# ProgramerSalar/stable-diffusion-from-scratch

Measured on NVIDIA B200. Metric: 512px DDIM-50 images/sec, higher is better.
Workload: dtype bf16

## Files before the change

include/sdb200.h:

```cpp
#ifndef SDB200_H
#define SDB200_H

#include <stdint.h>

#ifdef __cplusplus
extern "C" {
#endif

#define SDB_OK            0
#define SDB_ERR_INVALID  -1
#define SDB_ERR_CUDA     -2
#define SDB_ERR_NOTMA    -3

#define SDB_F32   0
#define SDB_BF16  1

int         sdb_version(void);
const char* sdb_last_error_string(void);
int         sdb_device_sm_count(void);
unsigned long long sdb_launch_count(void);
int sdb_pdl_skip_next(int n);

int sdb_nchw_to_nhwc(const float* src, void* dst, int dst_dtype, int N, int C, int dst_C, int HW, void* stream);
int sdb_nchw_to_nhwc_split(const float* src, void* dst , int N, int C, int dst_C, int HW, void* stream);
// ... 65 lines not shown
    long long lda, ldb, ldc, ldr, ldv;
    int M, N, K;
    float alpha;
    int b_kn;
    int nb1, nb2;
    long long sa1, sa2, sb1, sb2, sc1, sc2;
    int kh, kw, stride, pad, up;
    int NB, IH, IW, Cin, OH, OW;
    int out_dtype;
} sdb_simt_args;
int sdb_simt_contract(const sdb_simt_args* args , void* stream);

typedef struct sdb_tc_args {
    const void* A; const void* B; void* out;
    const float* bias; const float* rowvec; const float* residual;
    long long lda, ldb, ldc, ldr, ldv;
    int M, N, K;
    int out_dtype;
    int geglu;
    int col_group, col_group_stride;
    int split_k;
    int block_n;
    int taps;
    int kw;
    int stride, pad_h, pad_w;
    int NB, IH, IW, Cin, OH, OW;
    int cout_pad;
    int out_sh, out_sw, out_oh, out_ow, OHF, OWF;
    void* ws; long long ws_bytes;
    int rows_per_item;
    int variant;
    float* colstats; long long colstats_slots;
    int b_const;
} sdb_tc_args;
int sdb_tc_colstats_layout(const sdb_tc_args* args , long long* slots, long long* slots_per_item);
long long sdb_tc_workspace_bytes(const sdb_tc_args* args );
int sdb_tc_contract(const sdb_tc_args* args , void* stream);
int sdb_tc_set_pair_kernel(int enable);
int sdb_tc_set_tma_epilogue(int enable);
int sdb_tc_set_tail_split(int enable);

typedef struct sdb_attn_args {
    const void* q; const void* k; const void* v; void* out;
    long long q_bs, q_ss, q_hs;
    long long k_bs, k_ss, k_hs;
    long long v_bs, v_ss, v_hs;
    long long o_bs, o_ss, o_hs;
    int B, H, Sq, Sk, d, dpad;
    float scale;
    int dense;
    int causal;
} sdb_attn_args;
int sdb_attention_fwd(const sdb_attn_args* args , void* stream);
int sdb_attention_set_short_key_kernel(int enable);

int sdb_attention_wide_fwd(const void* q, const void* k, const void* v, void* out, long long q_bs, long long q_ss,
                           long long k_bs, long long k_ss, long long v_bs, long long v_ss, long long o_bs, long long o_ss,
                           int B, int Sq, int Sk, int d, float scale, void* stream);

#define SDB_NCHW  0
#define SDB_NHWC  1
long long sdb_vq_ws_bytes(long long M, int n_e);
int sdb_vq_quantize(const float* z, int z_layout, int N, int HW, int D, const float* codebook, int n_e, float beta,
                    float* z_q, int zq_layout, long long* idx, float* loss, void* ws, int* counters, void* stream);
int sdb_vq_codebook_gather(const long long* idx, long long M, const float* codebook, int n_e, int D, float* out, int out_layout,
                           int HW, void* stream);

int sdb_patch_unfold(const float* x, int B, int C, int H, int W, int kh, int kw, int sh, int sw, float* out, void* stream);
int sdb_patch_fold(const float* o, int B, int C, int KH, int KW, int Ly, int Lx, int SH, int SW, int OH, int OW,
                   const float* wpix, const float* wcrop, int L, float* out, void* stream);

#ifdef __cplusplus
}
// ... 3 lines not shown
```

stable-diffusion-from-scratch_b200/_lib.py:

```python
import ctypes as C
import os

import torch

HERE = os.path.dirname(os.path.abspath(__file__))
LIB_PATH = os.path.join(HERE, "libsdb200.so")

F32, BF16 = 0, 1

_lib = None


class SdbError(RuntimeError):
    pass


class SimtArgs(C.Structure):
    _fields_ = [
        ("A", C.c_void_p), ("B", C.c_void_p), ("out", C.c_void_p),
        ("bias", C.c_void_p), ("rowvec", C.c_void_p), ("residual", C.c_void_p),
        ("lda", C.c_longlong), ("ldb", C.c_longlong), ("ldc", C.c_longlong), ("ldr", C.c_longlong), ("ldv", C.c_longlong),
        ("M", C.c_int), ("N", C.c_int), ("K", C.c_int),
        ("alpha", C.c_float),
        ("b_kn", C.c_int),
        ("nb1", C.c_int), ("nb2", C.c_int),
        ("sa1", C.c_longlong), ("sa2", C.c_longlong), ("sb1", C.c_longlong), ("sb2", C.c_longlong),
        ("sc1", C.c_longlong), ("sc2", C.c_longlong),
        ("kh", C.c_int), ("kw", C.c_int), ("stride", C.c_int), ("pad", C.c_int), ("up", C.c_int),
        ("NB", C.c_int), ("IH", C.c_int), ("IW", C.c_int), ("Cin", C.c_int), ("OH", C.c_int), ("OW", C.c_int),
        ("out_dtype", C.c_int),
    ]


class TcArgs(C.Structure):
    _fields_ = [
        ("A", C.c_void_p), ("B", C.c_void_p), ("out", C.c_void_p),
        ("bias", C.c_void_p), ("rowvec", C.c_void_p), ("residual", C.c_void_p),
        ("lda", C.c_longlong), ("ldb", C.c_longlong), ("ldc", C.c_longlong), ("ldr", C.c_longlong), ("ldv", C.c_longlong),
        ("M", C.c_int), ("N", C.c_int), ("K", C.c_int),
        ("out_dtype", C.c_int),
        ("geglu", C.c_int),
        ("col_group", C.c_int), ("col_group_stride", C.c_int),
        ("split_k", C.c_int),
        ("block_n", C.c_int),
        ("taps", C.c_int), ("kw", C.c_int),
        ("stride", C.c_int), ("pad_h", C.c_int), ("pad_w", C.c_int),
        ("NB", C.c_int), ("IH", C.c_int), ("IW", C.c_int), ("Cin", C.c_int), ("OH", C.c_int), ("OW", C.c_int),
        ("cout_pad", C.c_int),
        ("out_sh", C.c_int), ("out_sw", C.c_int), ("out_oh", C.c_int), ("out_ow", C.c_int), ("OHF", C.c_int), ("OWF", C.c_int),
        ("ws", C.c_void_p), ("ws_bytes", C.c_longlong),
        ("rows_per_item", C.c_int),
        ("variant", C.c_int),
        ("colstats", C.c_void_p), ("colstats_slots", C.c_longlong),
        ("b_const", C.c_int),
    ]


class AttnArgs(C.Structure):
    _fields_ = [
        ("q", C.c_void_p), ("k", C.c_void_p), ("v", C.c_void_p), ("out", C.c_void_p),
        ("q_bs", C.c_longlong), ("q_ss", C.c_longlong), ("q_hs", C.c_longlong),
        ("k_bs", C.c_longlong), ("k_ss", C.c_longlong), ("k_hs", C.c_longlong),
        ("v_bs", C.c_longlong), ("v_ss", C.c_longlong), ("v_hs", C.c_longlong),
        ("o_bs", C.c_longlong), ("o_ss", C.c_longlong), ("o_hs", C.c_longlong),
        ("B", C.c_int), ("H", C.c_int), ("Sq", C.c_int), ("Sk", C.c_int), ("d", C.c_int), ("dpad", C.c_int),
        ("scale", C.c_float),
        ("dense", C.c_int),
        ("causal", C.c_int),
    ]


_P, _I, _L, _F = C.c_void_p, C.c_int, C.c_longlong, C.c_float
SIGNATURES = {
    "sdb_version": (_I, []),
    "sdb_last_error_string": (C.c_char_p, []),
    "sdb_device_sm_count": (_I, []),
    "sdb_launch_count": (C.c_ulonglong, []),
    "sdb_pdl_skip_next": (_I, [_I]),
    "sdb_nchw_to_nhwc": (_I, [_P, _P, _I, _I, _I, _I, _I, _P]),
    "sdb_nchw_to_nhwc_split": (_I, [_P, _P, _I, _I, _I, _I, _P]),
    "sdb_nchw_concat_to_nhwc": (_I, [_P, _I, _P, _I, _P, _I, _I, _I, _I, _I, _P]),
    "sdb_nhwc_to_nchw": (_I, [_P, _P, _I, _I, _I, _P]),
    "sdb_groupnorm_ws_bytes": (_L, [_I, _I, _I, _I]),
    "sdb_groupnorm_nhwc": (_I, [_P, _I, _P, _I, _I, _I, _I, _F, _P, _P, _L, _I, _I, _P, _I, _P, _P, _P, _P]),
    "sdb_scale_shift_affine": (_I, [_P, _P, _P, _L, _I, _I, _P, _P, _P]),
    "sdb_avgpool2x2": (_I, [_P, _I, _I, _I, _I, _P, _I, _P]),
    "sdb_groupnorm_from_colstats": (_I, [_P, _I, _P, C.POINTER(C.c_longlong), _P, _I, _P, C.POINTER(C.c_longlong), _I, _I, _I, _F,
                                         _P, _P, _L, _I, _I, _P, _I, _P, _P, _P]),
    "sdb_layernorm": (_I, [_P, _I, _I, _F, _P, _P, _P, _I, _P]),
    "sdb_cast_concat": (_I, [_P, _I, _P, _I, _I, _I, _I, _I, _P, _I, _P]),
    "sdb_upsample_bilinear2x": (_I, [_P, _I, _I, _I, _I, _P, _I, _P]),
    "sdb_activation": (_I, [_P, _P, _I, _L, _I, _P]),
    "sdb_geglu": (_I, [_P, _I, _I, _P, _I, _P]),
    "sdb_softmax_rows": (_I, [_P, _L, _I, _L, _F, _P, _I, _L, _P]),
    "sdb_softmax_rows_causal": (_I, [_P, _L, _I, _I, _L, _F, _P, _I, _L, _P]),
    "sdb_add": (_I, [_P, _P, _P, _L, _P]),
    "sdb_add_rowvec": (_I, [_P, _P, _L, _I, _L, _I, _P, _I, _P]),
    "sdb_timestep_embedding": (_I, [_P, _P, _I, _I, _I, _P, _P]),
    "sdb_gather_rows": (_I, [_P, _P, _I, _I, _P, _P]),
    "sdb_skinny_linear": (_I, [_P, _I, _I, _P, _P, _I, _I, _I, _P, _P]),
    "sdb_skinny_linear_bf16w": (_I, [_P, _I, _I, _P, _P, _I, _I, _I, _P, _P]),
    "sdb_ddim_step": (_I, [_P, _P, _P, _F, _P, _F, _F, _F, _F, _F, _F, _P, _P, _L, _P]),
    "sdb_ddim_xprev": (_I, [_P, _P, _P, _F, _P, _F, _F, _F, _F, _P, _L, _P]),
    "sdb_ddpm_step": (_I, [_P, _P, _P, _P, _P, _P, _I, _I, _F, _P, _P, _I, _L, _P]),
    "sdb_inpaint_blend": (_I, [_P, _P, _P, _P, _P, _P, _I, _I, _I, _L, _P, _P]),
    "sdb_diag_gaussian": (_I, [_P, _P, _I, _I, _L, _P, _P, _P, _P, _P, _P]),
    "sdb_q_sample": (_I, [_P, _P, _P, _P, _I, _L, _P, _P]),
    "sdb_simt_contract": (_I, [C.POINTER(SimtArgs), _P]),
    "sdb_tc_contract": (_I, [C.POINTER(TcArgs), _P]),
    "sdb_tc_set_pair_kernel": (_I, [_I]),
    "sdb_tc_set_tma_epilogue": (_I, [_I]),
    "sdb_tc_set_tail_split": (_I, [_I]),
    "sdb_tc_workspace_bytes": (_L, [C.POINTER(TcArgs)]),
    "sdb_tc_colstats_layout": (_I, [C.POINTER(TcArgs), C.POINTER(C.c_longlong), C.POINTER(C.c_longlong)]),
    "sdb_attention_fwd": (_I, [C.POINTER(AttnArgs), _P]),
    "sdb_attention_set_short_key_kernel": (_I, [_I]),
    "sdb_attention_wide_fwd": (_I, [_P, _P, _P, _P, _L, _L, _L, _L, _L, _L, _L, _L, _I, _I, _I, _I, _F, _P]),
    "sdb_vq_ws_bytes": (_L, [_L, _I]),
    "sdb_vq_quantize": (_I, [_P, _I, _I, _I, _I, _P, _I, _F, _P, _I, _P, _P, _P, _P, _P]),
    "sdb_vq_codebook_gather": (_I, [_P, _L, _P, _I, _I, _P, _I, _I, _P]),
    "sdb_patch_unfold": (_I, [_P, _I, _I, _I, _I, _I, _I, _I, _I, _P, _P]),
    "sdb_patch_fold": (_I, [_P, _I, _I, _I, _I, _I, _I, _I, _I, _I, _I, _P, _P, _I, _P, _P]),
}


def load(path=None):
    global _lib
    if _lib is not None and path is None:
        return _lib
    path = path or LIB_PATH
    if not os.path.exists(path):
        raise SdbError(
            "libsdb200.so not found at %s — build it with `python -c 'import __graft_entry__ as g; g.build()'`; "
            "there is no CPU or PyTorch fallback for the sdb200 hot path" % path)
    lib = C.CDLL(path)
    for name, (res, args) in SIGNATURES.items():
        fn = getattr(lib, name)
        fn.restype = res
        fn.argtypes = args
    _lib = lib
    return lib


def check(rc, what=""):
    if rc != 0:
# ... 39 lines not shown
```

stable-diffusion-from-scratch_b200/csrc/ptx.cuh:

```cuda
#pragma once
#include <cuda.h>
#include <stdint.h>

namespace sdb {
namespace ptx {

__device__ __forceinline__ uint32_t smem_u32(const void* p) {
    return static_cast<uint32_t>(__cvta_generic_to_shared(p));
}

__device__ __forceinline__ bool elect_one() {
    uint32_t pred;
    asm volatile(
        "{\n\t"
        ".reg .pred p;\n\t"
        "elect.sync _|p, 0xffffffff;\n\t"
        "selp.u32 %0, 1, 0, p;\n\t"
        "}"
        : "=r"(pred));
    return pred != 0;
}
__device__ __forceinline__ void mbar_init(uint64_t* bar, uint32_t count) {
    asm volatile("mbarrier.init.shared::cta.b64 [%0], %1;" ::"r"(smem_u32(bar)), "r"(count) : "memory");
}
// ... 236 lines not shown
__device__ __forceinline__ void umma_commit_pair(uint64_t* bar, uint16_t mask) {
    asm volatile("tcgen05.commit.cta_group::2.mbarrier::arrive::one.shared::cluster.multicast::cluster.b64 [%0], %1;"
                 ::"r"(smem_u32(bar)), "h"(mask) : "memory");
}

__device__ __forceinline__ void tma_store_5d(const CUtensorMap* tm, uint32_t src_smem, int c0, int c1, int c2, int c3, int c4) {
    asm volatile(
        "cp.async.bulk.tensor.5d.global.shared::cta.tile.bulk_group [%0, {%2, %3, %4, %5, %6}], [%1];"
        ::"l"(tm), "r"(src_smem), "r"(c0), "r"(c1), "r"(c2), "r"(c3), "r"(c4)
        : "memory");
}
__device__ __forceinline__ void tma_store_commit() { asm volatile("cp.async.bulk.commit_group;" ::: "memory"); }
template <int N>
__device__ __forceinline__ void tma_store_wait_read() { asm volatile("cp.async.bulk.wait_group.read %0;" ::"n"(N) : "memory"); }
template <int N>
__device__ __forceinline__ void tma_store_wait_all() { asm volatile("cp.async.bulk.wait_group %0;" ::"n"(N) : "memory"); }
__device__ __forceinline__ void tma_load_5d(uint32_t dst_smem, const CUtensorMap* tm, uint32_t bar_smem, int c0, int c1, int c2, int c3, int c4) {
    asm volatile(
        "cp.async.bulk.tensor.5d.shared::cluster.global.tile.mbarrier::complete_tx::bytes [%0], [%1, {%3, %4, %5, %6, %7}], [%2];"
        ::"r"(dst_smem), "l"(tm), "r"(bar_smem), "r"(c0), "r"(c1), "r"(c2), "r"(c3), "r"(c4)
        : "memory");
}
__device__ __forceinline__ void tma_prefetch_l2_5d(const CUtensorMap* tm, int c0, int c1, int c2, int c3, int c4) {
    asm volatile("cp.async.bulk.prefetch.tensor.5d.L2.global.tile [%0, {%1, %2, %3, %4, %5}];"
                 ::"l"(tm), "r"(c0), "r"(c1), "r"(c2), "r"(c3), "r"(c4) : "memory");
}
__device__ __forceinline__ void mbar_arrive_expect_tx_a(uint32_t bar_smem, uint32_t bytes) {
    asm volatile("mbarrier.arrive.expect_tx.shared::cta.b64 _, [%0], %1;" ::"r"(bar_smem), "r"(bytes) : "memory");
}
__device__ __forceinline__ void sts128f(uint32_t saddr, float a, float b, float c, float d) {
    asm volatile("st.shared.v4.f32 [%0], {%1,%2,%3,%4};" ::"r"(saddr), "f"(a), "f"(b), "f"(c), "f"(d) : "memory");
}

__device__ __forceinline__ void named_bar_sync(uint32_t id, uint32_t nthreads) {
    asm volatile("bar.sync %0, %1;" ::"r"(id), "r"(nthreads) : "memory");
}

}
}
```

stable-diffusion-from-scratch_b200/csrc/tc_contract.cu:

```cuda
#include "common.cuh"
#include "ptx.cuh"
#include <stdlib.h>
#include <string.h>

namespace sdb {

using namespace ptx;

struct TcP {
    void* out;
    const float* bias; const float* rowvec; const float* residual;
    float* ws; long long ws_split_stride;
    float* colstats; long long colstats_sq;
    long long ldc, ldr, ldv;
    int M, N;
    int kblocks;
    int kpt;
    int out_bf16, geglu;
    int col_group, col_group_stride;
    int split_k;
    int tiles_n;
    int m_pairs;
    int off32;
    int stages;
    int epi_tma;
    int epi_nbuf;
    int epi_bw, epi_bh;
    int b_const;
    int full_tiles;
    int conv;
    int kw, stride, pad_h, pad_w;
    int NB, OH, OW;
    int tw, th, tn, tiles_w, tiles_h;
    int cout_pad;
    int out_sh, out_sw, out_oh, out_ow, OHF, OWF;
#ifdef SDB_TC_TRACE
    long long* trace;
#endif
};

#ifdef SDB_TC_TRACE
#define TC_TRACE(slot, it_)                                                                              \
    do {                                                                                                 \
        if (p.trace && rank == 0 && (it_) < 64) p.trace[((long long)pair * 64 + (it_)) * 8 + (slot)] = clock64(); \
    } while (0)
static long long* g_trace_ptr = nullptr;
extern "C" void sdb_tc_set_trace(long long* ptr) { g_trace_ptr = ptr; }
#define TC1_TRACE(slot)                                                                                  \
    do {                                                                                                 \
        if (p.trace && blockIdx.x < 2048 && blockIdx.y == 0) {                                           \
            if ((slot) == 7) { unsigned sm; asm volatile("mov.u32 %0, %%smid;" : "=r"(sm)); p.trace[(long long)blockIdx.x * 8 + 7] = sm; } \
            else p.trace[(long long)blockIdx.x * 8 + (slot)] = (long long)globaltimer_ns();               \
        }                                                                                                \
    } while (0)
#else
#define TC_TRACE(slot, it_) do { } while (0)
#define TC1_TRACE(slot) do { } while (0)
#endif

constexpr int TC_BM = 128;
constexpr int TC_BK = 64;
// ... 299 lines not shown
                float* dst = p.colstats + (long long)slot * p.N + cn;
                *reinterpret_cast<float4*>(dst) = cs_s;
                *reinterpret_cast<float4*>(dst + p.colstats_sq) = cs_q;
            }
        }
    }
    __syncwarp();
}

template <int BN>
__device__ __forceinline__ void epilogue_warp(const TcP& p, uint32_t taddr, const float* s_bias, float* stage, int lane,
                                              int n0, int nt, long long row_pix, int row_img, int split, int ch0, int chstep,
                                              uint64_t* acc_ready, uint32_t acc_parity, int slot, int ncols = 1 << 30) {
    const int n_out = p.geglu ? p.N / 2 : p.N;
    const bool partial = p.split_k > 1;
    const bool fast_ok = p.off32 && (n_out % 4 == 0) && (p.ldc % 4 == 0) && (p.ldv % 4 == 0) &&
                         ((reinterpret_cast<uintptr_t>(p.out) | reinterpret_cast<uintptr_t>(p.residual) |
                           reinterpret_cast<uintptr_t>(p.rowvec) | reinterpret_cast<uintptr_t>(p.ws)) & 15) == 0 &&
                         (!p.col_group || (p.col_group % 4 == 0 && p.col_group_stride % 4 == 0)) &&
                         (p.residual == nullptr || partial || p.ldr == p.ldc) && !(p.geglu && (partial || !p.out_bf16));
#define SDB_EPI(MODE, ADD) epilogue_fast<BN, MODE, ADD>(p, taddr, s_bias, stage, lane, n0, nt, row_pix, row_img, split, ch0, chstep, acc_ready, acc_parity, slot, ncols)
    if (!fast_ok) {
        epilogue_generic<BN>(p, taddr, s_bias, stage, lane, n0, nt, row_pix, row_img, split, ch0, chstep, acc_ready, acc_parity, slot, ncols);
    } else if (p.geglu) {
        SDB_EPI(EPI_GEGLU, false);
    } else if (partial) {
        SDB_EPI(EPI_PARTIAL, false);
    } else {
        const bool has_add = p.residual != nullptr || (p.rowvec != nullptr && p.conv);
        if (p.out_bf16) { if (has_add) SDB_EPI(EPI_BF16, true); else SDB_EPI(EPI_BF16, false); }
        else            { if (has_add) SDB_EPI(EPI_F32, true);  else SDB_EPI(EPI_F32, false); }
    }
#undef SDB_EPI
}

struct UnitBox { int split, nt, mt, col0, w, h, n; };

template <int BN, int MODE, bool HAS_RES>
__device__ __forceinline__ void tepi_chunk(const TcP& p, const CUtensorMap* tmC, const uint32_t (&cur)[32], const uint32_t* g,
                                           uint32_t sb_a, uint32_t sbuf, int c0, int col, const UnitBox& ub, int lane, int lg,
                                           uint32_t rowmask, int img_w, bool rv_ok, const float* rowv, bool want_cs, bool partial,
                                           int n_out) {
    constexpr bool GEGLU = MODE == EPI_GEGLU;
    constexpr bool OUT16 = MODE != EPI_F32;
    if (OUT16) {
        const uint32_t rowa = sbuf + lane * 64;
        const uint32_t sw = (uint32_t)(lane >> 1) & 3u;
#pragma unroll
        for (int j = 0; j < 4; ++j) {
            float v[8];
#pragma unroll
            for (int h2 = 0; h2 < 2; ++h2) {
                const float4 b4 = lds128(sb_a + 4 * (c0 + 8 * j + 4 * h2));
                float x0 = __uint_as_float(cur[8 * j + 4 * h2 + 0]) + b4.x, x1 = __uint_as_float(cur[8 * j + 4 * h2 + 1]) + b4.y;
                float x2 = __uint_as_float(cur[8 * j + 4 * h2 + 2]) + b4.z, x3 = __uint_as_float(cur[8 * j + 4 * h2 + 3]) + b4.w;
                if (GEGLU) {
                    const float4 bg = lds128(sb_a + 4 * (BN / 2 + c0 + 8 * j + 4 * h2));
                    x0 *= gelu_erf_fast(__uint_as_float(g[(8 * j + 4 * h2 + 0) % (GEGLU ? 32 : 1)]) + bg.x);
                    x1 *= gelu_erf_fast(__uint_as_float(g[(8 * j + 4 * h2 + 1) % (GEGLU ? 32 : 1)]) + bg.y);
                    x2 *= gelu_erf_fast(__uint_as_float(g[(8 * j + 4 * h2 + 2) % (GEGLU ? 32 : 1)]) + bg.z);
                    x3 *= gelu_erf_fast(__uint_as_float(g[(8 * j + 4 * h2 + 3) % (GEGLU ? 32 : 1)]) + bg.w);
                }
                v[4 * h2 + 0] = x0; v[4 * h2 + 1] = x1; v[4 * h2 + 2] = x2; v[4 * h2 + 3] = x3;
            }
            sts128(rowa + ((((uint32_t)j) ^ sw) << 4), pack_bf16x2(v[0], v[1]), pack_bf16x2(v[2], v[3]), pack_bf16x2(v[4], v[5]),
                   pack_bf16x2(v[6], v[7]));
// ... 377 lines not shown
        } else {
            pix = (m0 + row) < p.M ? m0 + row : -1;
        }
        const uint32_t taddr = tmem_d + ((uint32_t)(lg * 32) << 16);
        if (p.epi_tma) {
            constexpr int NCH = BN / 32 > 0 ? BN / 32 : 1;
            UnitBox ub;
            ub.split = split; ub.nt = nt; ub.mt = mt; ub.col0 = p.geglu ? nt * (BN / 2) : n0;
            const int r0 = lg * 32;
            if (p.conv) {
                ub.w = ow0 + r0 % p.tw; ub.h = oh0 + (r0 / p.tw) % p.th; ub.n = img0 + r0 / (p.tw * p.th);
            } else {
                ub.w = m0 + r0; ub.h = 0; ub.n = 0;
            }
            const uint32_t rowmask = __ballot_sync(0xffffffffu, pix >= 0);
            const int img_w = __shfl_sync(0xffffffffu, img, 0);
            const uint32_t stg_a = smem_u32(sA) + (uint32_t)(warp - 2) * (uint32_t)(NCH * TEPI_BOX_BYTES);
            uint64_t* rbar = &res_bar[warp - 2];
#define SDB_TEPI1(MODE, RES) epilogue_tma_single<BN, MODE, RES>(p, &tmC, &tmR, taddr, smem_u32(s_bias), stg_a, rbar, accum_bar, ub, lane, lg, rowmask, img_w, ncols)
            if (p.geglu) {
                if constexpr (BN % 64 == 0) SDB_TEPI1(EPI_GEGLU, false);
            } else if (p.split_k > 1) SDB_TEPI1(EPI_F32, false);
            else if (p.out_bf16) SDB_TEPI1(EPI_BF16, false);
            else if (p.residual != nullptr) SDB_TEPI1(EPI_F32, true);
            else SDB_TEPI1(EPI_F32, false);
#undef SDB_TEPI1
        } else {
            prefetch_residual_row(p, pix, n0, BN);
            float* stage = reinterpret_cast<float*>(sA) + (warp - 2) * (EPI_WARP_BYTES / 4);
            if (warp == 2 && lane == 0) TC1_TRACE(4);
            epilogue_warp<BN>(p, taddr, s_bias, stage, lane, n0, nt, pix, img, split, 0, 1, accum_bar, 0, mt * 4 + lg, ncols);
            if (warp == 2 && lane == 0) TC1_TRACE(5);
        }
    }

    tcgen05_fence_before();
    __syncthreads();
    if (warp == 1) {
        tcgen05_fence_after();
        tmem_dealloc(tmem_d, Cfg::TMEM_COLS);
    }
}

constexpr int TC2_MAX_STAGES = 8;
constexpr int TC2_SMEM_LIMIT = 232448;

template <int BN, int EW>
struct Tc2Cfg {
    static constexpr int THREADS = 128 + 32 * EW;
    static constexpr int B_HALF_BYTES = (BN / 2) * TC_BK * 2;
    static constexpr int STAGE_BYTES = TC_A_BYTES + B_HALF_BYTES;
    static constexpr int ACC_STRIDE = 256;
    static constexpr int FIXED_BYTES = 1024 + 512 + 2 * BN * 4 + 1024;
    __host__ __device__ static constexpr int staging_bytes(int epi_tma, int nbuf) { return epi_tma ? EW * nbuf * TEPI_BOX_BYTES : EW * EPI_WARP_BYTES; }
    __host__ static int stages_for(int staging) {
        int st = (TC2_SMEM_LIMIT - FIXED_BYTES - staging) / STAGE_BYTES;
        return st > TC2_MAX_STAGES ? TC2_MAX_STAGES : st;
    }
    __host__ static int smem_bytes(int stages, int staging) { return FIXED_BYTES + stages * STAGE_BYTES + staging; }
};

template <int BN, int EW>
__global__ void __cluster_dims__(2, 1, 1) __launch_bounds__(128 + 32 * EW, 1)
tc_contract_pair_kernel(const __grid_constant__ CUtensorMap tmA, const __grid_constant__ CUtensorMap tmB,
                        const __grid_constant__ CUtensorMap tmC, const __grid_constant__ CUtensorMap tmR, const TcP p) {
    pdl_trigger();
// ... 316 lines not shown
}

template <int BN>
static int launch_tc_pair(const CUtensorMap& tmA, const CUtensorMap& tmB, const CUtensorMap& tmC, const CUtensorMap& tmR, TcP& p,
                          int m_tiles, cudaStream_t st) {
#ifdef SDB_TC_EW16
    static int forced = -1;
    if (forced < 0) { const char* e = getenv("SDB200_TC_EW"); forced = e ? atoi(e) : 0; }
    if (forced == 16) return launch_tc_pair_ew<BN, 16>(tmA, tmB, tmC, tmR, p, m_tiles, st);
#endif
    return launch_tc_pair_ew<BN, 8>(tmA, tmB, tmC, tmR, p, m_tiles, st);
}

static int g_pair_kernel = -1;
static bool pair_kernel_enabled() {
    if (g_pair_kernel < 0) {
        const char* e = getenv("SDB200_TC_KERNEL");
        g_pair_kernel = (e && strcmp(e, "single") == 0) ? 0 : 1;
    }
    return g_pair_kernel == 1;
}

static int g_tail_split = -1;
static bool tail_split_enabled() {
    if (g_tail_split < 0) { const char* e = getenv("SDB200_TC_TAILSPLIT"); g_tail_split = (e && e[0] == '0') ? 0 : 1; }
    return g_tail_split == 1;
}

static int g_tma_epilogue = -1;
static bool tma_epilogue_enabled() {
    if (g_tma_epilogue < 0) { const char* e = getenv("SDB200_TC_EPI"); g_tma_epilogue = (e && strcmp(e, "regs") == 0) ? 0 : 1; }
    return g_tma_epilogue == 1;
}
static int tma_epilogue_max_kblocks() {
    static int v = -1;
    if (v < 0) { const char* e = getenv("SDB200_TC_EPI_MAXKB"); v = e ? atoi(e) : 40; }
    return v;
}

struct ReduceRemap { int on, OH, OW, sh, sw, oh0, ow0, OHF, OWF; };

__global__ void splitk_reduce_kernel(const float* __restrict__ ws, long long split_stride, int splits, long long rows, int N,
                                     const float* __restrict__ bias, const float* __restrict__ rowvec, long long ldv,
                                     long long rows_per_img, const float* __restrict__ residual, long long ldr,
                                     void* __restrict__ out, long long ldc, int out_bf16, const ReduceRemap rm) {
    pdl_trigger();
    pdl_wait();
    const int nq = N >> 2;
    const long long total = rows * nq;
    for (long long i = (long long)blockIdx.x * blockDim.x + threadIdx.x; i < total; i += (long long)gridDim.x * blockDim.x) {
        long long m = i / nq;
        const int n = (int)(i - m * nq) << 2;
        if (rm.on) {
            const long long img = m / ((long long)rm.OH * rm.OW);
            const int rem = (int)(m - img * rm.OH * rm.OW);
            const int oh = rem / rm.OW, ow = rem - oh * rm.OW;
            m = (img * rm.OHF + (oh * rm.sh + rm.oh0)) * rm.OWF + (ow * rm.sw + rm.ow0);
        }
        float4 acc = *reinterpret_cast<const float4*>(ws + m * N + n);
        for (int s = 1; s < splits; ++s) {
            float4 q = *reinterpret_cast<const float4*>(ws + s * split_stride + m * N + n);
            acc.x += q.x; acc.y += q.y; acc.z += q.z; acc.w += q.w;
        }
        if (bias) { acc.x += bias[n]; acc.y += bias[n + 1]; acc.z += bias[n + 2]; acc.w += bias[n + 3]; }
        if (rowvec) {
            const float* rp = rowvec + (m / rows_per_img) * ldv + n;
// ... 137 lines not shown
            }
        }
    }
    if (sk < 1) sk = 1;
    if (sk > pl->kblocks) sk = pl->kblocks;
    SDB_REQUIRE(sk == 1 || splittable, "tc_contract: split_k needs a plain (no GEGLU / column remap) output with N %% 4 == 0");
    pl->split_k = sk;
    pl->ws_bytes = sk > 1 ? (long long)sk * pl->rows_out * a->N * 4 : 0;
    return SDB_OK;
}

}

using namespace sdb;

extern "C" int sdb_tc_set_pair_kernel(int enable) {
    int prev = pair_kernel_enabled() ? 1 : 0;
    g_pair_kernel = enable ? 1 : 0;
    return prev;
}

extern "C" int sdb_tc_set_tail_split(int enable) {
    int prev = tail_split_enabled() ? 1 : 0;
    g_tail_split = enable ? 1 : 0;
    return prev;
}

extern "C" int sdb_tc_set_tma_epilogue(int enable) {
    int prev = tma_epilogue_enabled() ? 1 : 0;
    g_tma_epilogue = enable ? 1 : 0;
    return prev;
}

extern "C" long long sdb_tc_workspace_bytes(const sdb_tc_args* a) {
    if (!a) return -1;
    sdb_tc_args t = *a;
    if (t.split_k == 0 && !t.ws) t.ws = reinterpret_cast<void*>(16);
    TcPlan pl;
    if (make_plan(&t, &pl) != SDB_OK) return -1;
    return pl.ws_bytes;
}

static bool colstats_supported(const sdb_tc_args* a, const TcPlan& pl) {
    if (!(a->taps > 0 && !a->geglu && !a->col_group && a->out_dtype == SDB_F32 && a->N % 4 == 0 && a->ldc % 4 == 0)) return false;
    if (pl.split_k > 1) return a->out_sh <= 1 && ((long long)a->OH * a->OW) % 32 == 0 && (a->OHF <= 0 || a->OHF == a->OH) && (a->OWF <= 0 || a->OWF == a->OW);
    return pl.tn == 1 || (pl.tiles_w * pl.tiles_h == 1 && pl.tw * pl.th >= 32);
}

static void colstats_layout(const sdb_tc_args* a, const TcPlan& pl, long long* slots, long long* slots_per_item) {
    if (pl.split_k > 1) {
        *slots = pl.rows_out / 32;
        *slots_per_item = ((long long)a->OH * a->OW) / 32;
    } else {
        const long long mt = pl.use_pair ? 2LL * ((pl.m_tiles + 1) / 2) : pl.m_tiles;
        *slots = 4 * mt;
        *slots_per_item = 4LL * pl.tiles_w * pl.tiles_h / pl.tn;
    }
}

extern "C" int sdb_tc_colstats_layout(const sdb_tc_args* a, long long* slots, long long* slots_per_item) {
    if (!a || !slots || !slots_per_item) return SDB_ERR_INVALID;
    *slots = 0; *slots_per_item = 0;
    sdb_tc_args t = *a;
    if (t.split_k == 0 && !t.ws) t.ws = reinterpret_cast<void*>(16);
    TcPlan pl;
    int rc = make_plan(&t, &pl);
    if (rc) return rc;
    if (!colstats_supported(a, pl)) return SDB_OK;
    colstats_layout(a, pl, slots, slots_per_item);
    return SDB_OK;
}

extern "C" int sdb_tc_contract(const sdb_tc_args* a, void* stream) {
    SDB_REQUIRE(a && a->A && a->B && a->out, "tc_contract: null pointer");
    TcPlan pl;
    int rc = make_plan(a, &pl);
    if (rc) return rc;
    if (a->colstats) {
        SDB_REQUIRE(colstats_supported(a, pl), "tc_contract: column statistics need an fp32 conv output whose 32-row slots lie inside one sample");
        long long need_slots = 0, spi_ = 0;
        colstats_layout(a, pl, &need_slots, &spi_);
        SDB_REQUIRE(a->colstats_slots >= need_slots, "tc_contract: colstats buffer has %lld slots, needs %lld", a->colstats_slots, need_slots);
        SDB_REQUIRE(((uintptr_t)a->colstats & 15) == 0 && ((uintptr_t)a->out & 15) == 0 && (!a->residual || (((uintptr_t)a->residual & 15) == 0 && a->ldr % 4 == 0)) &&
                    (!a->rowvec || (((uintptr_t)a->rowvec & 15) == 0 && a->ldv % 4 == 0)), "tc_contract: column statistics need 16-byte aligned operands");
    }
    const bool conv = a->taps > 0;
    const int bn = pl.bn;
    const bool use_pair = pl.use_pair;

    TcP p;
    memset(&p, 0, sizeof(p));
    p.out = a->out; p.bias = a->bias; p.rowvec = a->rowvec; p.residual = a->residual;
    p.ldc = a->ldc; p.ldr = a->ldr; p.ldv = a->ldv;
    p.M = a->M; p.N = a->N;
    p.kpt = pl.kpt;
    p.b_const = a->b_const ? 1 : 0;
    p.kblocks = pl.kblocks;
    p.out_bf16 = a->out_dtype == SDB_BF16;
    p.geglu = a->geglu;
    p.col_group = a->col_group; p.col_group_stride = a->col_group_stride;
    p.split_k = pl.split_k;
    if (p.split_k > 1) {
        SDB_REQUIRE(a->ws && a->ws_bytes >= pl.ws_bytes, "tc_contract: split_k=%d needs a %lld-byte workspace (got %lld)",
                    p.split_k, pl.ws_bytes, a->ws ? a->ws_bytes : 0LL);
        SDB_REQUIRE(((uintptr_t)a->ws & 15) == 0, "tc_contract: workspace must be 16-byte aligned");
        p.ws = reinterpret_cast<float*>(a->ws);
        p.ws_split_stride = pl.rows_out * a->N;
    }
    {
        const long long ld_max = a->ldc > a->N ? a->ldc : a->N;
        p.off32 = (pl.rows_out + 1) * ld_max + a->N < (1LL << 32) ? 1 : 0;
    }
    p.colstats = pl.split_k > 1 ? nullptr : a->colstats;
    p.colstats_sq = a->colstats ? a->colstats_slots * (long long)a->N : 0;
#ifdef SDB_TC_TRACE
    p.trace = g_trace_ptr;
#endif
    p.tiles_n = pl.tiles_n;
    p.conv = conv;
    p.cout_pad = conv ? a->cout_pad : 0;

    CUtensorMap tmA, tmB;
    const int m_tiles = pl.m_tiles;
    const int taps = pl.taps;
    if (conv) {
        p.tw = pl.tw; p.th = pl.th; p.tn = pl.tn;
        p.kw = a->kw; p.stride = a->stride; p.pad_h = a->pad_h; p.pad_w = a->pad_w;
        p.NB = a->NB; p.OH = a->OH; p.OW = a->OW;
        p.tiles_w = pl.tiles_w; p.tiles_h = pl.tiles_h;
        p.out_sh = a->out_sh > 0 ? a->out_sh : 1; p.out_sw = a->out_sw > 0 ? a->out_sw : 1;
        p.out_oh = a->out_oh; p.out_ow = a->out_ow;
        p.OHF = a->OHF > 0 ? a->OHF : a->OH; p.OWF = a->OWF > 0 ? a->OWF : a->OW;
        long long ldx = a->lda > 0 ? a->lda : a->Cin;
        long long dims[4] = {a->Cin, a->IW, a->IH, a->NB};
        long long strides[3] = {ldx, ldx * a->IW, ldx * a->IW * a->IH};
        int box[4] = {TC_BK, p.tw * a->stride, p.th * a->stride, p.tn};
        int es[4] = {1, a->stride, a->stride, 1};
        rc = make_tmap_bf16(&tmA, a->A, 4, dims, strides, box, es);
        if (rc) return rc;
        long long bdims[2] = {a->Cin, (long long)taps * a->cout_pad};
        long long bstr[1] = {a->ldb > 0 ? a->ldb : a->Cin};
        int bbox[2] = {TC_BK, use_pair ? bn / 2 : bn};
        int bes[2] = {1, 1};
        rc = make_tmap_bf16(&tmB, a->B, 2, bdims, bstr, bbox, bes);
        if (rc) return rc;
    } else {
// ... 46 lines not shown
            rc = make_tmap(&tmC, obase, ebytes, out16 ? 64 : 128, 5, dims, str, box, es5);
            if (rc == SDB_OK && has_res) {
                const long long ldr = a->ldr;
                dims[4] = 1;
                if (conv) { str[0] = ldr; str[1] = ldr * p.OW; str[2] = ldr * p.OW * p.OH; str[3] = ldr * p.OW * p.OH * p.NB; }
                else { str[0] = ldr; str[1] = ldr * a->M; str[2] = ldr * a->M; str[3] = ldr * a->M; }
                rc = make_tmap(&tmR, a->residual, 4, 128, 5, dims, str, box, es5);
            }
            if (rc == SDB_OK) {
                p.epi_tma = 1;
                p.epi_bw = bw; p.epi_bh = bh;
                p.epi_nbuf = has_res ? (kb_split <= 24 ? 3 : 2) : 2;
            } else {
                rc = SDB_OK;
            }
        }
    }
    if (!p.epi_tma) p.epi_nbuf = 0;
    if (use_pair) {
        switch (bn) {
            case 128: rc = launch_tc_pair<128>(tmA, tmB, tmC, tmR, p, m_tiles, st); break;
            case 160: rc = launch_tc_pair<160>(tmA, tmB, tmC, tmR, p, m_tiles, st); break;
            default: rc = launch_tc_pair<256>(tmA, tmB, tmC, tmR, p, m_tiles, st); break;
        }
    } else {
        switch (bn) {
            case 32: rc = launch_tc<32>(tmA, tmB, tmC, tmR, p, m_tiles, st); break;
            case 64: rc = launch_tc<64>(tmA, tmB, tmC, tmR, p, m_tiles, st); break;
            case 128: rc = launch_tc<128>(tmA, tmB, tmC, tmR, p, m_tiles, st); break;
            case 160: rc = launch_tc<160>(tmA, tmB, tmC, tmR, p, m_tiles, st); break;
            default: rc = launch_tc<256>(tmA, tmB, tmC, tmR, p, m_tiles, st); break;
        }
    }
    if (rc || p.split_k == 1) return rc;
    ReduceRemap rm;
    memset(&rm, 0, sizeof(rm));
    long long red_rows = pl.rows_out;
    if (conv && (p.out_sh != 1 || p.out_sw != 1 || p.out_oh != 0 || p.out_ow != 0 || p.OHF != p.OH || p.OWF != p.OW)) {
        rm.on = 1; rm.OH = p.OH; rm.OW = p.OW; rm.sh = p.out_sh; rm.sw = p.out_sw; rm.oh0 = p.out_oh; rm.ow0 = p.out_ow;
        rm.OHF = p.OHF; rm.OWF = p.OWF;
        red_rows = (long long)p.NB * p.OH * p.OW;
    }
    const long long total = red_rows * (a->N / 4);
    int blocks = (int)((total + 255) / 256);
    if (blocks > 148 * 8) blocks = 148 * 8;
    const long long rows_per_img = conv ? (long long)p.OHF * p.OWF : 1;
    if (a->colstats) {
        SDB_REQUIRE(!p.out_bf16 && ((uintptr_t)a->out & 15) == 0 && a->ldc % 4 == 0 && (!a->bias || ((uintptr_t)a->bias & 15) == 0),
                    "tc_contract: split-K column statistics need 16-byte aligned fp32 operands");
        dim3 g((unsigned)(pl.rows_out / 32), (unsigned)((a->N / 4 + 31) / 32));
        launch_pdl(splitk_reduce_stats_kernel, dim3(g), dim3(256), 0, st, p.ws, p.ws_split_stride, p.split_k, pl.rows_out, a->N, a->bias,
                   conv ? a->rowvec : nullptr, a->ldv, rows_per_img, a->residual, a->ldr, reinterpret_cast<float*>(a->out), a->ldc,
                   a->colstats, p.colstats_sq);
        return check_launch("splitk_reduce_stats_kernel");
    }
    launch_pdl(splitk_reduce_kernel, dim3(blocks), dim3(256), 0, st, p.ws, p.ws_split_stride, p.split_k, red_rows, a->N, a->bias,
                                                 conv ? a->rowvec : nullptr, a->ldv, rows_per_img, a->residual, a->ldr,
                                                 a->out, a->ldc, p.out_bf16, rm);
    return check_launch("splitk_reduce_kernel");
}
```

stable-diffusion-from-scratch_b200/ops.py:

```python
import ctypes as C
import os

import torch

from . import _lib
from ._lib import BF16, F32, AttnArgs, SimtArgs, TcArgs, check, dtype_code, ptr, require_cuda, stream_ptr


def _L():
    return _lib.load()


def nchw_to_nhwc(x, out_dtype=torch.float32, pad_to=0, split=False, x1=None):
    require_cuda(x, x1)
    assert x.dtype == torch.float32 and x.is_contiguous()
    N, Cc, H, W = x.shape
    C1 = 0
    if x1 is not None:
        assert x1.dtype == torch.float32 and x1.is_contiguous() and x1.dim() == 4
        assert x1.shape[0] == N and tuple(x1.shape[2:]) == (H, W), "nchw_to_nhwc: x1 %s does not match x %s" % (
            tuple(x1.shape), tuple(x.shape))
        C1 = x1.shape[1]
    Ct = Cc + C1
    Cd = max(Ct, pad_to)
# ... 475 lines not shown
    a.kh = 0
    a.out_dtype = dtype_code(out.dtype)
    check(_L().sdb_simt_contract(C.byref(a), stream_ptr()), "simt gemm")
    return out


def _plan_table():
    if os.environ.get("SDB200_TC_PLANS", "1") == "0":
        return {}
    from .tc_plans import PLANS
    return PLANS


_PLANS = None


def _apply_plan(a, kind, rows_per_sample):
    global _PLANS
    if a.split_k or a.variant or (a.block_n and not a.geglu):
        return
    if _PLANS is None:
        _PLANS = _plan_table()
    key = (kind, int(rows_per_sample), a.N, a.K, a.taps, a.stride if a.taps else 0, a.geglu, int(bool(a.residual)),
           a.out_dtype, a.col_group)
    hit = _PLANS.get(key)
    if hit is not None:
        if a.geglu:
            if hit[1] == a.block_n:
                a.variant = hit[0]
        else:
            a.variant, a.block_n, a.split_k = hit[0], hit[1], hit[2]


def _tc_launch(a, what):
    lib = _L()
    need = lib.sdb_tc_workspace_bytes(C.byref(a))
    if need < 0:
        check(-1, what)
    ws = None
    if need > 0:
        ws = torch.empty(need, dtype=torch.uint8, device=torch.device("cuda", torch.cuda.current_device()))
        a.ws, a.ws_bytes = ws.data_ptr(), need
    check(lib.sdb_tc_contract(C.byref(a), stream_ptr()), what)


def conv_tc(x, w_rskc, bias, kh, kw, stride=1, pad=0, rowvec=None, residual=None, out_dtype=torch.float32,
            split_k=0, block_n=0, out=None, phase=None, variant=0, want_stats=False, stats_into=None, pad_hi=None, b_const=False):
    require_cuda(x, w_rskc, bias, rowvec, residual, out)
    assert x.dtype == torch.bfloat16 and w_rskc.dtype == torch.bfloat16 and x.is_contiguous() and w_rskc.is_contiguous()
    N, IH, IW, Cin = x.shape
    taps, Cout, Cin2 = w_rskc.shape
    assert Cin2 == Cin and taps == kh * kw
    a = TcArgs()
    if phase is None:
        pad_hi = pad if pad_hi is None else pad_hi
        OH = (IH + pad + pad_hi - kh) // stride + 1
        OW = (IW + pad + pad_hi - kw) // stride + 1
        pad_h = pad_w = pad
        if out is None:
            out = torch.empty((N, OH, OW, Cout), dtype=out_dtype, device=x.device)
        a.out_sh = a.out_sw = 1
        a.out_oh = a.out_ow = 0
        a.OHF, a.OWF = OH, OW
    else:
        sh, sw, o_h, o_w, OHF, OWF, pad_h, pad_w = phase
        OH, OW = IH, IW
        assert out is not None and tuple(out.shape) == (N, OHF, OWF, Cout)
        a.out_sh, a.out_sw, a.out_oh, a.out_ow, a.OHF, a.OWF = sh, sw, o_h, o_w, OHF, OWF
    a.A, a.B, a.out = ptr(x), ptr(w_rskc), ptr(out)
    a.bias, a.rowvec, a.residual = ptr(bias), ptr(rowvec), ptr(residual)
    a.lda, a.ldb, a.ldc = Cin, Cin, Cout
    a.ldr = Cout
    a.ldv = rowvec.stride(0) if rowvec is not None else 0
    a.M, a.N, a.K = N * OH * OW, Cout, taps * Cin
    a.out_dtype = dtype_code(out.dtype)
# ... 159 lines not shown
```

Measured before the change: 14.60.

## Fuse split-K reduction into GEMM epilogue via per-tile arrival counters

Adds an in-kernel split-K fixup. Each split writes its partial tile to the workspace, then increments a per-tile atomic counter. The last-arriving CTA sums the partials and applies bias, rowvec, residual and column statistics, so the separate split-K reduce kernel launch is skipped. This removes a kernel launch and one extra pass over the workspace, at the cost of a serialized tail in the last CTA per tile, atomics and fences, and a persistent counter buffer that resets itself. It applies only when split_k is at most 3 and the tile is small enough; otherwise the reduce kernel still runs.

```diff
diff --git a/include/sdb200.h b/include/sdb200.h
--- a/include/sdb200.h
+++ b/include/sdb200.h
@@ -121,13 +121,16 @@
     int variant;
     float* colstats; long long colstats_slots;
     int b_const;
+    int* tile_ctr; long long tile_ctr_len;
 } sdb_tc_args;
 int sdb_tc_colstats_layout(const sdb_tc_args* args , long long* slots, long long* slots_per_item);
 long long sdb_tc_workspace_bytes(const sdb_tc_args* args );
+long long sdb_tc_tile_counters(const sdb_tc_args* args );
 int sdb_tc_contract(const sdb_tc_args* args , void* stream);
 int sdb_tc_set_pair_kernel(int enable);
 int sdb_tc_set_tma_epilogue(int enable);
 int sdb_tc_set_tail_split(int enable);
+int sdb_tc_set_splitk_fixup(int enable);
 
 typedef struct sdb_attn_args {
     const void* q; const void* k; const void* v; void* out;
diff --git a/stable-diffusion-from-scratch_b200/_lib.py b/stable-diffusion-from-scratch_b200/_lib.py
--- a/stable-diffusion-from-scratch_b200/_lib.py
+++ b/stable-diffusion-from-scratch_b200/_lib.py
@@ -53,6 +53,7 @@
         ("variant", C.c_int),
         ("colstats", C.c_void_p), ("colstats_slots", C.c_longlong),
         ("b_const", C.c_int),
+        ("tile_ctr", C.c_void_p), ("tile_ctr_len", C.c_longlong),
     ]
 
 
@@ -111,6 +112,8 @@
     "sdb_tc_set_pair_kernel": (_I, [_I]),
     "sdb_tc_set_tma_epilogue": (_I, [_I]),
     "sdb_tc_set_tail_split": (_I, [_I]),
+    "sdb_tc_set_splitk_fixup": (_I, [_I]),
+    "sdb_tc_tile_counters": (_L, [C.POINTER(TcArgs)]),
     "sdb_tc_workspace_bytes": (_L, [C.POINTER(TcArgs)]),
     "sdb_tc_colstats_layout": (_I, [C.POINTER(TcArgs), C.POINTER(C.c_longlong), C.POINTER(C.c_longlong)]),
     "sdb_attention_fwd": (_I, [C.POINTER(AttnArgs), _P]),
diff --git a/stable-diffusion-from-scratch_b200/csrc/ptx.cuh b/stable-diffusion-from-scratch_b200/csrc/ptx.cuh
--- a/stable-diffusion-from-scratch_b200/csrc/ptx.cuh
+++ b/stable-diffusion-from-scratch_b200/csrc/ptx.cuh
@@ -292,6 +292,13 @@
     asm volatile("st.shared.v4.f32 [%0], {%1,%2,%3,%4};" ::"r"(saddr), "f"(a), "f"(b), "f"(c), "f"(d) : "memory");
 }
 
+__device__ __forceinline__ void fence_proxy_async_global() { asm volatile("fence.proxy.async.global;" ::: "memory"); }
+__device__ __forceinline__ int atom_add_acq_rel_gpu(int* p, int v) {
+    int old;
+    asm volatile("atom.add.acq_rel.gpu.global.s32 %0, [%1], %2;" : "=r"(old) : "l"(p), "r"(v) : "memory");
+    return old;
+}
+
 __device__ __forceinline__ void named_bar_sync(uint32_t id, uint32_t nthreads) {
     asm volatile("bar.sync %0, %1;" ::"r"(id), "r"(nthreads) : "memory");
 }
diff --git a/stable-diffusion-from-scratch_b200/csrc/tc_contract.cu b/stable-diffusion-from-scratch_b200/csrc/tc_contract.cu
--- a/stable-diffusion-from-scratch_b200/csrc/tc_contract.cu
+++ b/stable-diffusion-from-scratch_b200/csrc/tc_contract.cu
@@ -27,6 +27,7 @@
     int epi_nbuf;
     int epi_bw, epi_bh;
     int b_const;
+    int* tile_ctr;
     int full_tiles;
     int conv;
     int kw, stride, pad_h, pad_w;
@@ -392,6 +393,136 @@
         else            { if (has_add) SDB_EPI(EPI_F32, true);  else SDB_EPI(EPI_F32, false); }
     }
 #undef SDB_EPI
+}
+
+__device__ __forceinline__ long long tile_row_pix(const TcP& p, int mt, int row, int& img) {
+    img = 0;
+    if (p.conv) {
+        const int tww = mt % p.tiles_w, thh = (mt / p.tiles_w) % p.tiles_h, tnb = mt / (p.tiles_w * p.tiles_h);
+        const int in_ = row / (p.th * p.tw), rem = row - in_ * (p.th * p.tw);
+        const int ih = rem / p.tw, iw = rem - ih * p.tw;
+        img = tnb * p.tn + in_;
+        const int oh = thh * p.th + ih, ow = tww * p.tw + iw;
+        const bool valid = img < p.NB && oh < p.OH && ow < p.OW;
+        return valid ? ((long long)img * p.OHF + (oh * p.out_sh + p.out_oh)) * p.OWF + (ow * p.out_sw + p.out_ow) : -1;
+    }
+    return mt * TC_BM + row < p.M ? (long long)mt * TC_BM + row : -1;
+}
+
+constexpr int TC_FIXUP_MAX_SPLIT = 3;
+constexpr long long TC_FIXUP_MAX_BYTES = 96 * 1024;
+
+__device__ __forceinline__ void f4_add(float4& a, const float4& b) { a.x += b.x; a.y += b.y; a.z += b.z; a.w += b.w; }
+
+__device__ __noinline__ void splitk_fixup(const TcP p , int mt, int nt, int n0, int ncols, int ew,
+                                          int lane, volatile int* s_ticket, uint32_t bar_id) {
+    constexpr int NW = 4;
+    tma_store_wait_all<0>();
+    fence_proxy_async_global();
+    __threadfence();
+    named_bar_sync(bar_id, 32 * NW);
+    if (ew == 0 && lane == 0) {
+        int* ctr = p.tile_ctr + ((long long)mt * p.tiles_n + nt);
+        const bool last = atom_add_acq_rel_gpu(ctr, 1) == p.split_k - 1;
+        if (last) *ctr = 0;
+        *s_ticket = last ? 1 : 0;
+    }
+    named_bar_sync(bar_id, 32 * NW);
+    if (*s_ticket == 0) return;
+    __threadfence();
+
+    int img;
+    const long long pix = tile_row_pix(p, mt, ew * 32 + lane, img);
+    const float* const rowv = p.conv ? p.rowvec : nullptr;
+    const bool cs_on = p.colstats != nullptr;
+    const bool vec = ((p.ldc | p.ldr | p.ldv) & 3) == 0 &&
+                     ((reinterpret_cast<uintptr_t>(p.out) | reinterpret_cast<uintptr_t>(p.residual) |
+                       reinterpret_cast<uintptr_t>(rowv) | reinterpret_cast<uintptr_t>(p.bias)) & 15) == 0;
+    const long long pix0 = __shfl_sync(0xffffffffu, pix, 0);
+    const int npass = (ncols + 127) / 128;
+#pragma unroll 1
+    for (int c = 0; c < npass; ++c) {
+        const int cc = c * 128 + 4 * lane;
+        const int col = n0 + cc;
+        const bool col_ok = cc < ncols && col < p.N;
+        float4 b4 = make_float4(0.f, 0.f, 0.f, 0.f);
+        if (p.bias && col_ok) b4 = make_float4(__ldg(p.bias + col), __ldg(p.bias + col + 1), __ldg(p.bias + col + 2), __ldg(p.bias + col + 3));
+        float4 t_s = make_float4(0.f, 0.f, 0.f, 0.f), t_q = make_float4(0.f, 0.f, 0.f, 0.f);
+#pragma unroll 1
+        for (int g = 0; g < 8; ++g) {
+            long long pr[4];
+            int ir[4];
+#pragma unroll
+            for (int i = 0; i < 4; ++i) {
+                pr[i] = __shfl_sync(0xffffffffu, pix, 4 * g + i);
+                ir[i] = __shfl_sync(0xffffffffu, img, 4 * g + i);
+                if (!col_ok) pr[i] = -1;
+            }
+            float4 v[TC_FIXUP_MAX_SPLIT][4];
+#pragma unroll
+            for (int s = 0; s < TC_FIXUP_MAX_SPLIT; ++s)
+#pragma unroll
+                for (int i = 0; i < 4; ++i)
+                    v[s][i] = (s < p.split_k && pr[i] >= 0)
+                                  ? __ldcg(reinterpret_cast<const float4*>(p.ws + s * p.ws_split_stride + pr[i] * p.N + col))
+                                  : make_float4(0.f, 0.f, 0.f, 0.f);
+            float4 rsd[4], tev[4];
+#pragma unroll
+            for (int i = 0; i < 4; ++i) {
+                rsd[i] = tev[i] = make_float4(0.f, 0.f, 0.f, 0.f);
+                if (pr[i] < 0) continue;
+                if (rowv) {
+                    const float* rp = rowv + (long long)ir[i] * p.ldv + col;
+                    tev[i] = vec ? __ldg(reinterpret_cast<const float4*>(rp)) : make_float4(__ldg(rp), __ldg(rp + 1), __ldg(rp + 2), __ldg(rp + 3));
+                }
+                if (p.residual) {
+                    const float* rp = p.residual + pr[i] * p.ldr + col;
+                    rsd[i] = vec ? __ldg(reinterpret_cast<const float4*>(rp)) : make_float4(__ldg(rp), __ldg(rp + 1), __ldg(rp + 2), __ldg(rp + 3));
+                }
+            }
+            float4 acc[4];
+#pragma unroll
+            for (int i = 0; i < 4; ++i) {
+                acc[i] = v[0][i];
+#pragma unroll
+                for (int s = 1; s < TC_FIXUP_MAX_SPLIT; ++s)
+                    if (s < p.split_k) f4_add(acc[i], v[s][i]);
+            }
+            float4 g_s = make_float4(0.f, 0.f, 0.f, 0.f), g_q = make_float4(0.f, 0.f, 0.f, 0.f);
+#pragma unroll
+            for (int i = 0; i < 4; ++i) {
+                if (pr[i] < 0) continue;
+                float4 a = acc[i];
+                if (cs_on || p.bias) f4_add(a, b4);
+                if (rowv) f4_add(a, tev[i]);
+                if (p.residual) f4_add(a, rsd[i]);
+                if (p.out_bf16) {
+                    __nv_bfloat16* o = reinterpret_cast<__nv_bfloat16*>(p.out) + pr[i] * p.ldc + col;
+                    if (vec) {
+                        *reinterpret_cast<uint2*>(o) = make_uint2(pack_bf16x2(a.x, a.y), pack_bf16x2(a.z, a.w));
+                    } else {
+                        o[0] = __float2bfloat16_rn(a.x); o[1] = __float2bfloat16_rn(a.y);
+                        o[2] = __float2bfloat16_rn(a.z); o[3] = __float2bfloat16_rn(a.w);
+                    }
+                } else {
+                    float* o = reinterpret_cast<float*>(p.out) + pr[i] * p.ldc + col;
+                    if (vec) *reinterpret_cast<float4*>(o) = a;
+                    else { o[0] = a.x; o[1] = a.y; o[2] = a.z; o[3] = a.w; }
+                }
+                if (cs_on) {
+                    f4_add(g_s, a);
+                    g_q.x = fmaf(a.x, a.x, g_q.x); g_q.y = fmaf(a.y, a.y, g_q.y); g_q.z = fmaf(a.z, a.z, g_q.z); g_q.w = fmaf(a.w, a.w, g_q.w);
+                }
+            }
+            if (g == 0) { t_s = g_s; t_q = g_q; }
+            else { f4_add(t_s, g_s); f4_add(t_q, g_q); }
+        }
+        if (cs_on && col_ok && pix0 >= 0) {
+            float* dst = p.colstats + (pix0 / 32) * p.N + col;
+            *reinterpret_cast<float4*>(dst) = t_s;
+            *reinterpret_cast<float4*>(dst + p.colstats_sq) = t_q;
+        }
+    }
 }
 
 struct UnitBox { int split, nt, mt, col0, w, h, n; };
@@ -835,6 +966,8 @@
             epilogue_warp<BN>(p, taddr, s_bias, stage, lane, n0, nt, pix, img, split, 0, 1, accum_bar, 0, mt * 4 + lg, ncols);
             if (warp == 2 && lane == 0) TC1_TRACE(5);
         }
+        if (p.split_k > 1 && p.tile_ctr)
+            splitk_fixup(p, mt, nt, n0, ncols, warp - 2, lane, reinterpret_cast<volatile int*>(res_bar + 4), 2);
     }
 
     tcgen05_fence_before();
@@ -1217,6 +1350,11 @@
     if (g_tma_epilogue < 0) { const char* e = getenv("SDB200_TC_EPI"); g_tma_epilogue = (e && strcmp(e, "regs") == 0) ? 0 : 1; }
     return g_tma_epilogue == 1;
 }
+static int g_splitk_fixup = -1;
+static bool splitk_fixup_enabled() {
+    if (g_splitk_fixup < 0) { const char* e = getenv("SDB200_TC_SPLITK"); g_splitk_fixup = (e && strcmp(e, "reduce") == 0) ? 0 : 1; }
+    return g_splitk_fixup == 1;
+}
 static int tma_epilogue_max_kblocks() {
     static int v = -1;
     if (v < 0) { const char* e = getenv("SDB200_TC_EPI_MAXKB"); v = e ? atoi(e) : 40; }
@@ -1420,6 +1558,12 @@
     return prev;
 }
 
+extern "C" int sdb_tc_set_splitk_fixup(int enable) {
+    int prev = splitk_fixup_enabled() ? 1 : 0;
+    g_splitk_fixup = enable ? 1 : 0;
+    return prev;
+}
+
 extern "C" long long sdb_tc_workspace_bytes(const sdb_tc_args* a) {
     if (!a) return -1;
     sdb_tc_args t = *a;
@@ -1433,6 +1577,23 @@
     if (!(a->taps > 0 && !a->geglu && !a->col_group && a->out_dtype == SDB_F32 && a->N % 4 == 0 && a->ldc % 4 == 0)) return false;
     if (pl.split_k > 1) return a->out_sh <= 1 && ((long long)a->OH * a->OW) % 32 == 0 && (a->OHF <= 0 || a->OHF == a->OH) && (a->OWF <= 0 || a->OWF == a->OW);
     return pl.tn == 1 || (pl.tiles_w * pl.tiles_h == 1 && pl.tw * pl.th >= 32);
+}
+
+static long long tile_counters(const TcPlan& pl) {
+    if (pl.split_k <= 1 || pl.use_pair || pl.split_k > TC_FIXUP_MAX_SPLIT || (long long)pl.split_k * TC_BM * pl.bn * 4 > TC_FIXUP_MAX_BYTES)
+        return 0;
+    return (long long)pl.m_tiles * pl.tiles_n;
+}
+
+static bool fixup_colstats_ok(const sdb_tc_args* a, const TcPlan& pl) {
+    return a->taps > 0 && pl.tw == a->OW && (pl.tn == 1 || pl.th == a->OH);
+}
+
+extern "C" long long sdb_tc_tile_counters(const sdb_tc_args* a) {
+    if (!a) return -1;
+    TcPlan pl;
+    if (make_plan(a, &pl) != SDB_OK) return -1;
+    return tile_counters(pl);
 }
 
 static void colstats_layout(const sdb_tc_args* a, const TcPlan& pl, long long* slots, long long* slots_per_item) {
@@ -1499,7 +1660,15 @@
         const long long ld_max = a->ldc > a->N ? a->ldc : a->N;
         p.off32 = (pl.rows_out + 1) * ld_max + a->N < (1LL << 32) ? 1 : 0;
     }
-    p.colstats = pl.split_k > 1 ? nullptr : a->colstats;
+    if (p.split_k > 1 && a->colstats)
+        SDB_REQUIRE(!p.out_bf16 && ((uintptr_t)a->out & 15) == 0 && a->ldc % 4 == 0 && (!a->bias || ((uintptr_t)a->bias & 15) == 0),
+                    "tc_contract: split-K column statistics need 16-byte aligned fp32 operands");
+    if (tile_counters(pl) > 0 && splitk_fixup_enabled() && a->tile_ctr && a->tile_ctr_len >= tile_counters(pl) &&
+        (!a->colstats || fixup_colstats_ok(a, pl))) {
+        SDB_REQUIRE(((uintptr_t)a->tile_ctr & 3) == 0, "tc_contract: tile counters must be 4-byte aligned");
+        p.tile_ctr = a->tile_ctr;
+    }
+    p.colstats = (pl.split_k > 1 && !p.tile_ctr) ? nullptr : a->colstats;
     p.colstats_sq = a->colstats ? a->colstats_slots * (long long)a->N : 0;
 #ifdef SDB_TC_TRACE
     p.trace = g_trace_ptr;
@@ -1612,7 +1781,7 @@
             default: rc = launch_tc<256>(tmA, tmB, tmC, tmR, p, m_tiles, st); break;
         }
     }
-    if (rc || p.split_k == 1) return rc;
+    if (rc || p.split_k == 1 || p.tile_ctr) return rc;
     ReduceRemap rm;
     memset(&rm, 0, sizeof(rm));
     long long red_rows = pl.rows_out;
@@ -1626,8 +1795,6 @@
     if (blocks > 148 * 8) blocks = 148 * 8;
     const long long rows_per_img = conv ? (long long)p.OHF * p.OWF : 1;
     if (a->colstats) {
-        SDB_REQUIRE(!p.out_bf16 && ((uintptr_t)a->out & 15) == 0 && a->ldc % 4 == 0 && (!a->bias || ((uintptr_t)a->bias & 15) == 0),
-                    "tc_contract: split-K column statistics need 16-byte aligned fp32 operands");
         dim3 g((unsigned)(pl.rows_out / 32), (unsigned)((a->N / 4 + 31) / 32));
         launch_pdl(splitk_reduce_stats_kernel, dim3(g), dim3(256), 0, st, p.ws, p.ws_split_stride, p.split_k, pl.rows_out, a->N, a->bias,
                    conv ? a->rowvec : nullptr, a->ldv, rows_per_img, a->residual, a->ldr, reinterpret_cast<float*>(a->out), a->ldc,
diff --git a/stable-diffusion-from-scratch_b200/ops.py b/stable-diffusion-from-scratch_b200/ops.py
--- a/stable-diffusion-from-scratch_b200/ops.py
+++ b/stable-diffusion-from-scratch_b200/ops.py
@@ -531,6 +531,21 @@
             a.variant, a.block_n, a.split_k = hit[0], hit[1], hit[2]
 
 
+_tc_counters = {}
+_tc_counters_retired = []
+
+
+def _tc_counter_buffer(dev, n):
+    key = (dev.index, torch.cuda.current_stream(dev).cuda_stream)
+    buf = _tc_counters.get(key)
+    if buf is None or buf.numel() < n:
+        if buf is not None:
+            _tc_counters_retired.append(buf)
+        buf = torch.zeros(max(n, 16384), dtype=torch.int32, device=dev)
+        _tc_counters[key] = buf
+    return buf
+
+
 def _tc_launch(a, what):
     lib = _L()
     need = lib.sdb_tc_workspace_bytes(C.byref(a))
@@ -538,8 +553,15 @@
         check(-1, what)
     ws = None
     if need > 0:
-        ws = torch.empty(need, dtype=torch.uint8, device=torch.device("cuda", torch.cuda.current_device()))
+        dev = torch.device("cuda", torch.cuda.current_device())
+        ws = torch.empty(need, dtype=torch.uint8, device=dev)
         a.ws, a.ws_bytes = ws.data_ptr(), need
+        nctr = lib.sdb_tc_tile_counters(C.byref(a))
+        if nctr < 0:
+            check(-1, what)
+        if nctr > 0:
+            ctr = _tc_counter_buffer(dev, nctr)
+            a.tile_ctr, a.tile_ctr_len = ctr.data_ptr(), ctr.numel()
     check(lib.sdb_tc_contract(C.byref(a), stream_ptr()), what)
 
 
```

Result: no change. 14.46 (median of 6 runs) (-1.0%).
